# MarkJhonBao/InfantPoseEstimation_GaussianBias

Hardware: AMD Instinct MI355X
Metric: images/sec (train fwd+bwd) HRFormer-S 256x192 (higher is better)
Workload: dtype bf16; 1 GPU; HRFormer-small + fusion head, 256x192 -> 64x48, K=17, train step fwd+bwd+AdamW, DropPath 0.1, BN train; global_batch=64, per_gpu_batch=64, parallelism=dp1, launch=hipGraph replay, branches on concurrent HIP streams

## Files before the change

include/posekernels.h:

```cpp
#ifndef POSEKERNELS_H
#define POSEKERNELS_H

#include <stdint.h>

#ifdef __cplusplus
extern "C" {
#endif

#define PK_OK 0
#define PK_ERR_INVALID (-1)
#define PK_ERR_UNSUPPORTED (-2)

#define PK_DT_F32 0
#define PK_DT_BF16 1

int pk_version(void);
const char* pk_last_error_string(void);
int pk_marker(int id, void* stream);

int pk_gaussian_target(const float* keypoints, const float* visible, const float* lut, int lut_len,
                       float* target, float* weight, int B, int K, int Hh, int Wh,
                       double stride_x, double stride_y, double reach, int patch_n, int patch_c, void* stream);

int pk_dense_target(const float* keypoints, const float* visible, float* heatmaps, float* weights,
// ... 219 lines not shown
} PkConvDesc;
int pk_conv2d_group(const PkConvDesc* descs, int n, void* stream);
typedef struct PkBnFwdDesc {
    const void* raw; const float* stats_partial; const float* gamma; const float* beta;
    float* running_mean; float* running_var; int64_t* num_batches_tracked;
    const void* residual; void* y; float* save_mean; float* save_rstd; uint8_t* relu_mask ;
    int64_t rows; int tiles, C; float momentum, eps; int relu;
} PkBnFwdDesc;
int pk_bn_train_fwd_group(const PkBnFwdDesc* descs, int n, void* stream);
typedef struct PkBnBwdDesc {
    const void* dy; const void* y_act; const void* raw; const float* save_mean; const float* save_rstd; const float* gamma;
    float* partial; float* dgamma; float* dbeta; void* dx; void* dresidual; const uint8_t* relu_mask ;
    int64_t rows; int C; int relu;
} PkBnBwdDesc;
int pk_bn_bwd_group_blocks(int64_t rows);
int pk_bn_bwd_group(const PkBnBwdDesc* descs, int n, void* stream);
typedef struct PkFuseDesc {
    const void* inputs[4]; int in_h[4]; int in_w[4]; int n_inputs;
    void* out; const void* mask_y; int B, H, W, C, relu;
} PkFuseDesc;
int pk_fuse_sum_group(const PkFuseDesc* descs, int n, void* stream);
typedef struct PkUpBwdDesc {
    const void* dy; const void* mask_y; void* dsrc; int B, H, W, Hs, Ws, C;
} PkUpBwdDesc;
int pk_upsample_bwd_group(const PkUpBwdDesc* descs, int n, void* stream);
typedef struct PkWgradDesc {
    const void* x; const void* grad_out; float* workspace;
    int B, Hs, Ws, Ho, Wo, N, Cin, ksize, stride;
} PkWgradDesc;
int pk_wgrad_group_slices(int M, int N, int Cin, int ksize, int stride);
int pk_wgrad_group(const PkWgradDesc* descs, int n, void* stream);
int pk_sizeof_group_desc(int which);

int pk_conv_stats_rows(int B, int Hs, int Ws, int Cin, int Cout, int ksize, int stride, int Ho, int Wo);

int pk_linear_bf16(const void* x, const void* w, void* out, const float* bias, const void* residual, const float* res_scale,
                   const int32_t* a_rowmap, const int32_t* o_rowmap, void* preact_out, const void* gelu_grad_of,
                   int M, int N, int K, int rows_per_sample, int act, int out_fp32, void* stream);

int pk_rows_by_map(const void* src, void* dst, const int32_t* rowmap, int64_t n_rows, int row_bytes, int scatter, void* stream);
int pk_drop_path_f32(const float* x, const float* mask, float* out, int64_t batch, int64_t per_sample, float keep_prob, void* stream);

int pk_wgrad_slices(int M, int N, int Cin, int ksize, int stride, int Hs, int Ws, int flags);
int pk_wgrad_bf16(const void* x, const void* grad_out, float* workspace, float* dw, float* dbias, int n_bias,
                  const int32_t* a_rowmap, const int32_t* g_rowmap, const float* g_scale, int g_rows_per_sample, int M, int N,
                  int Cin, int ksize, int stride, int B, int Hs, int Ws, int Ho, int Wo, int out_layout, void* stream);

int pk_window_attn_fwd(const void* qkv, const float* rel_table, void* out, float* lse, int n_windows, int heads, int C,
                       float softmax_scale, void* stream);
int pk_window_attn_bwd_groups(int n_windows, int heads);
int pk_window_attn_bwd_ws_floats(int n_windows, int heads);
int pk_window_attn_bwd(const void* qkv, const float* rel_table, const void* fwd_out, const void* dout, const float* lse, void* dqkv,
                       float* dbias_partial, float* dtable, int n_windows, int heads, int C, float softmax_scale, void* stream);

int pk_sum_partials(const float* partial, int nb, int K, int stride, float* out, float scale, int accumulate, void* stream);
int pk_bn_finalize(const float* stats_partial, int tiles, int C, int count, const float* gamma, const float* beta,
                   float* running_mean, float* running_var, int64_t* num_batches_tracked, float momentum, float eps,
                   float* scale, float* shift, float* save_mean, float* save_rstd, void* stream);
int pk_bn_act(const void* x, const float* scale, const float* shift, const void* residual, void* y, int64_t rows, int C,
              int relu, uint8_t* relu_mask, void* stream);
int pk_bn_train_fwd(const void* raw, const float* stats_partial, int tiles, int C, int64_t rows, const float* gamma, const float* beta,
                    float* running_mean, float* running_var, int64_t* num_batches_tracked, float momentum, float eps, const void* residual,
                    void* y, float* save_mean, float* save_rstd, float* scale, float* shift, int relu, uint8_t* relu_mask, void* stream);
int pk_bn_bwd_blocks(int64_t rows);
int pk_bn_bwd(const void* dy, const void* y_act, const void* raw, const float* save_mean, const float* save_rstd,
              const float* gamma, float* partial, float* sums, float* dgamma, float* dbeta, void* dx, void* dresidual,
              int64_t rows, int C, int relu, const uint8_t* relu_mask, void* stream);
int pk_relu_bwd(const void* dy, const void* y, void* dx, int64_t numel, void* stream);

int pk_conv1x1_bn_supported(int64_t rows, int Cin, int Cout);
int pk_conv1x1_stats_rows(int64_t rows);
int pk_conv1x1_bn_bwd_rows(int64_t rows);
int pk_conv1x1_stats(const void* x, const void* w, float* stats_partial, int64_t rows, int Cin, int Cout, void* stream);
int pk_conv1x1_bn_act(const void* x, const void* w, const float* scale, const float* shift, const void* residual, void* y, int relu,
                      uint8_t* relu_mask, int64_t rows, int Cin, int Cout, void* stream);
int pk_conv1x1_bn_bwd_reduce(const void* dy, const void* x, const void* w, const float* save_mean, const float* save_rstd, float* partial,
                             int64_t rows, int Cin, int Cout, int relu, const uint8_t* relu_mask, void* stream);
int pk_conv1x1_bn_bwd_apply(const void* dy, const void* x, const void* w, const float* save_mean, const float* save_rstd, const float* gamma,
                            const float* sums, float inv_count, void* draw, void* dresidual, int64_t rows, int Cin, int Cout, int relu,
                            const uint8_t* relu_mask, void* stream);
int pk_conv1x1_bn_bwd(const void* dy, const void* x, const void* w, const float* save_mean, const float* save_rstd, const float* gamma,
                      float* partial, float* sums, float* dgamma, float* dbeta, void* draw, void* dresidual, int64_t rows, int Cin, int Cout,
                      int relu, const uint8_t* relu_mask, void* stream);
int pk_layernorm_fwd(const void* x, const float* gamma, const float* beta, void* y, float* save_mean, float* save_rstd,
                     int64_t rows, int C, int C_real, float eps, void* stream);
int pk_ln_bwd_blocks(int64_t rows);
int pk_layernorm_bwd(const void* dy, const void* x, const float* save_mean, const float* save_rstd, const float* gamma,
                     const void* dresidual, void* dx, float* partial, float* dgamma, float* dbeta, int64_t rows, int C, int C_real,
                     void* stream);
int pk_ln_mlp_supported(int C);
int pk_ln_mlp_hidden_slice(int C);
int pk_ln_mlp_slab_floats(int C);
int pk_ln_mlp_dx_blocks(int M, int C);
int pk_ln_mlp_dw_blocks(int M, int C);
int pk_ln_mlp_fwd(const void* x, const float* gamma, const float* beta, const void* w1, const float* b1, const void* w2,
                  const float* b2, const float* row_scale, void* y, int M, int C, int rows_per_sample, float eps, void* stream);
int pk_ln_mlp_wide_supported(int C, int hidden, int M);
int pk_ln_mlp_wide_fwd(const void* x, const float* gamma, const float* beta, const void* w1, const float* b1, const void* w2,
                       const float* b2, const float* row_scale, void* y, int M, int C, int c_real, int hidden, int rows_per_sample,
                       float eps, void* stream);
int pk_ln_mlp_bwd_dx(const void* dy, const void* x, const float* gamma, const float* beta, const void* w1, const float* b1,
                     const void* w1_t, const void* w2_t, const float* row_scale, void* dx, float* ln_partial, int M, int C,
                     int rows_per_sample, float eps, void* stream);
int pk_ln_mlp_bwd_dw(const void* dy, const void* x, const float* gamma, const float* beta, const void* w1, const float* b1,
                     const void* w2_t, const float* row_scale, float* slabs, int M, int C, int rows_per_sample, float eps,
                     void* stream);
int pk_attn_block_wide_supported(int C, int heads, int n_windows);
int pk_attn_block_wide_fwd(const void* x, const int32_t* rowmap, const float* gamma, const float* beta, const float* rel_table,
                           const void* wqkv, const float* bqkv, const void* wproj, const float* bproj, const float* row_scale,
                           void* y, int n_windows, int windows_per_sample, int heads, int C, int c_real, float softmax_scale,
                           float eps, void* stream);
int pk_attn_block_supported(int C, int heads);
int pk_attn_block_fwd(const void* x, const int32_t* rowmap, const float* gamma, const float* beta, const float* rel_table,
                      const void* wqkv, const float* bqkv, const void* wproj, const float* bproj, const float* row_scale,
                      void* y, void* o_save, float* lse, int n_windows, int windows_per_sample, int heads, int C, float eps,
                      void* stream);
int pk_attn_block_blocks(int n_windows);
int pk_attn_block_bwd(const void* dy, const void* x, const int32_t* rowmap, const float* gamma, const float* beta,
                      const float* rel_table, const void* wqkv, const float* bqkv, const void* wqkv_t, const void* wproj_t,
                      const float* row_scale, const void* o_saved, const float* lse, void* dx, void* dqkv, void* u_out,
                      float* ln_partial, float* rpb_partial, int n_windows, int windows_per_sample, int heads, int C, float eps,
                      void* stream);
int pk_colsum_bf16(const void* g, const int32_t* rowmap, const float* row_scale, int rows_per_sample, float* partial,
                   float* out, int64_t rows, int N, void* stream);
int pk_fuse_sum(const void* const* inputs, const int* in_h, const int* in_w, int n_inputs, void* out, int B, int H, int W,
                int C, int relu, void* stream);
int pk_upsample_bilinear_bwd(const void* dy, void* dsrc, int B, int H, int W, int Hs, int Ws, int C, void* stream);
int pk_nchw_f32_to_nhwc_bf16(const float* x, const float* softplus_out, void* y, int B, int Cin, int H, int W, int Cpad,
                             void* stream);
int pk_reduce_many_cols(void);
int pk_reduce_many(const void* desc_table, const int* block_desc, const int* block_first, int n_blocks, void* stream);
int pk_pack_weights(void* flat_dst_bf16, const void* desc_table, const int32_t* block_desc, const int32_t* block_first,
                    int n_blocks, void* stream);
int pk_embed_boxes(float* twin_base, const void* desc_table, const int* block_desc, const int* block_first, int n_blocks,
                   int direction, void* stream);

int pk_draw_shapes(void* images_u8, int N, int H, int W, const float* poses, const float* scores, const int32_t* image_index, int P,
                   int K, const int32_t* limbs, int L, const void* colors_u8, int C, const float* boxes,
                   const int32_t* box_image_index, int Q, int box_c0, int box_c1, int box_c2, int box_thickness,
                   float score_threshold, int point_radius, int line_thickness, void* stream);
int pk_heatmap_overlay_ws_floats(int N, int K, int h, int w, int H, int W);
int pk_heatmap_overlay(void* images_u8, const float* heatmaps, float alpha, const void* lut_u8, void* index_u8, float* ws, int N,
                       int K, int h, int w, int H, int W, void* stream);
int pk_heatmap_overlay_patches_ws_floats(int P, int K, int h, int w);
int pk_heatmap_overlay_patches(void* images_u8, const float* heatmaps, const int32_t* patch_image_index, const double* patch_matrix,
                               float alpha, const void* lut_u8, void* index_u8, void* cover_u8, float* ws, int N, int P, int K, int h,
                               int w, int H, int W, void* stream);

#ifdef __cplusplus
}
#endif
#endif
```

infantposeestimation_gaussianbias_amd/dispatch.py:

```python
import contextlib
import os

import torch

from . import nnops
from ._lib import PoseKernelError

_ACTIVE = []


def backend_for(model):
    ok = getattr(model, "_pk_supported", None)
    if ok is None:
        ok = nnops.supported(model)
        object.__setattr__(model, "_pk_supported", ok)
    if not ok:
        raise PoseKernelError(
            f"{type(model).__name__}: layer shapes outside the HIP kernels (channels must be multiples of 8, head_dim a multiple of 8 "
            "up to 64, window 7) and no 8-aligned padded twin could be built (models/padded.py); there is no fallback path")
    return nnops


def padded_twin(model):
    if getattr(model, "_pk_twin", None) is False:
        return None
    from .models import padded
    return padded.twin_for(model)


def backend_name(model) -> str:
    if torch.cuda.is_available() and padded_twin(model) is not None:
        return "hip (8-aligned padded twin)"
    backend_for(model)
    return "hip"


@contextlib.contextmanager
def scope(model):
    if _ACTIVE:
        yield _ACTIVE[-1]
        return
    ops = backend_for(model)
    _ACTIVE.append(ops)
    try:
        with nnops.use_weights(model):
            yield ops
            join_detached()
    finally:
        _ACTIVE.pop()


def ops():
    if not _ACTIVE:
        raise RuntimeError("network op called outside dispatch.scope(model)")
    return _ACTIVE[-1]


from .nnops import (backward_milestone, conv_bn_act, deconv_bn_relu, drop_scales, eval_drop_scales, exchange, exchange_output, head_out,
                    mlp_rows, residual_block, stochastic_depth, to_features, window_attention_tokens, window_block)


def to_public(x):
    ops()
    return x.permute(0, 3, 1, 2)


def from_public(x):
    ops()
    if x.dtype != nnops.ACT_DTYPE:
        B, C, H, W = x.shape
        if x.requires_grad and torch.is_grad_enabled() and C % 8 == 0:
            return x.permute(0, 2, 3, 1).to(nnops.ACT_DTYPE).contiguous()
        return nnops.to_features(x, cpad=-(-C // 8) * 8)
    return x.permute(0, 2, 3, 1).contiguous()


_SIDE = {}
_STREAMS_OFF = [False]
_REGION = [False]
_EVENTS = []


def set_streams(enabled: bool):
    _STREAMS_OFF[0] = not enabled


def set_region_mode(enabled: bool):
    _REGION[0] = bool(enabled)


def streams_enabled() -> bool:
    return (not _STREAMS_OFF[0]) and os.environ.get("POSE_STREAMS", "1") != "0" and torch.cuda.is_available()


def _side_stream(dev, i):
    key = (dev.index if dev.index is not None else torch.cuda.current_device(), i)
    if key not in _SIDE:
        _SIDE[key] = torch.cuda.Stream(device=dev)
    return _SIDE[key]


def join_side_streams(cur=None):
    cur = cur or torch.cuda.current_stream()
    for s in _SIDE.values():
        cur.wait_stream(s)


_DETACHED = []


def run_detached(fn, tensors):
    with torch.no_grad():
        if not streams_enabled() or _MARK:
            fn()
            return
        cur = torch.cuda.current_stream()
        s = _side_stream(cur.device, 7)
        _order(cur, s)
        with torch.cuda.stream(s):
            for t in tensors:
                t.record_stream(s)
            fn()
        _DETACHED.append(s)


def join_detached():
    if _DETACHED:
        cur = torch.cuda.current_stream()
        for s in _DETACHED:
            _order(s, cur)
        _DETACHED.clear()




def _tensors(obj):
    if torch.is_tensor(obj):
        yield obj
    elif isinstance(obj, (list, tuple)):
        for o in obj:
            yield from _tensors(o)
# ... 129 lines not shown
```

infantposeestimation_gaussianbias_amd/models/fusion_head.py:

```python
import math
from typing import Dict, Optional, Tuple

import torch
import torch.nn as nn

from .. import hipops
from .. import dispatch as nnops
from ._blocks import conv
from .losses import HardKeypointMining


class SoftArgmax2D(nn.Module):

    def __init__(self, beta: float = 1.0):
        super().__init__()
        self.beta = beta

    def forward(self, heatmaps: torch.Tensor) -> Tuple[torch.Tensor, torch.Tensor]:
        h = heatmaps.float()
        if torch.is_grad_enabled() and h.requires_grad:
            co, sc = hipops.softargmax(h)
            if self.beta != 1.0:
                co = hipops.softargmax(h * self.beta)[0]
            return co, sc
        one = torch.full((1,), 40.0, device=heatmaps.device)
        co, sc = hipops.softargmax_refine_decode(h, None, one, None, radius=0)
        if self.beta != 1.0:
            co, _ = hipops.softargmax_refine_decode((h * self.beta).contiguous(), None, one, None, radius=0)
        return co, sc


class LocalGaussianRefinement(nn.Module):

    def __init__(self, local_radius: int = 2):
        super().__init__()
        self.local_radius = local_radius

    @torch.no_grad()
    def forward(self, heatmaps: torch.Tensor, coarse_coords: torch.Tensor) -> torch.Tensor:
        return hipops.local_gaussian_refine(heatmaps.float(), coarse_coords.float(), self.local_radius)


class SubPixelRefinement(nn.Module):

    def __init__(self, beta: float = 1.0, local_radius: int = 2, fusion_alpha: float = 0.5):
        super().__init__()
        self.local_radius = local_radius
        self.soft_argmax = SoftArgmax2D(beta=beta)
        self.local_refine = LocalGaussianRefinement(local_radius=local_radius)
        self.alpha = nn.Parameter(torch.tensor(fusion_alpha))

    def forward(self, heatmaps):
        return hipops.softargmax_refine_decode(heatmaps.float(), None, self.alpha.detach(), None, self.local_radius)


def _branch(cin, hidden, cout):
    seq = nn.ModuleDict({"0": conv(cin, hidden, 3), "1": nn.BatchNorm2d(hidden), "3": nn.Conv2d(hidden, cout, 1)})
    return seq


class HeatmapRegressionHead(nn.Module):
    def __init__(self, in_channels: int, num_keypoints: int = 17, hidden_dim: int = 256, use_subpixel_refinement: bool = True):
        super().__init__()
        self.in_channels, self.num_keypoints, self.use_subpixel_refinement = in_channels, num_keypoints, use_subpixel_refinement
        self.shared_layers = nn.ModuleDict({"0": conv(in_channels, hidden_dim, 3), "1": nn.BatchNorm2d(hidden_dim),
                                            "3": conv(hidden_dim, hidden_dim, 3), "4": nn.BatchNorm2d(hidden_dim)})
        self.heatmap_branch = _branch(hidden_dim, hidden_dim, num_keypoints)
        self.offset_branch = _branch(hidden_dim, hidden_dim, num_keypoints * 2)
        self.variance_branch = _branch(hidden_dim, hidden_dim // 2, num_keypoints)
        if use_subpixel_refinement:
            self.subpixel_refine = SubPixelRefinement(1.0, 2, 0.5)
        self.fusion_weight = nn.Parameter(torch.tensor(0.5))
        for m in self.modules():
            if isinstance(m, nn.Conv2d):
                nn.init.kaiming_normal_(m.weight, mode="fan_out", nonlinearity="relu")
                if m.bias is not None:
                    nn.init.zeros_(m.bias)

    def forward(self, x: torch.Tensor) -> Dict[str, torch.Tensor]:
        with nnops.scope(self):
            return self._forward(x)

    def _forward(self, x: torch.Tensor) -> Dict[str, torch.Tensor]:
        tr = self.training
        x = nnops.from_public(x)
        s = self.shared_layers
        f = nnops.conv_bn_act(x, s["0"], s["1"], True, None, tr)
        f = nnops.conv_bn_act(f, s["3"], s["4"], True, None, tr)

        def make(br, softplus=False):
            def run(ins):
                t = nnops.conv_bn_act(ins[0], br["0"], br["1"], True, None, tr)
                return nnops.head_out(t, br["3"], softplus)
            return run

        heatmaps, offsets, variances = nnops.parallel([make(self.heatmap_branch), make(self.offset_branch), make(self.variance_branch, True)],
                                                      [[f], [f], [f]])
        B, _, H, W = offsets.shape
        return {"heatmaps": heatmaps, "offsets": offsets.view(B, self.num_keypoints, 2, H, W),
                "variances": variances, "fusion_weight": torch.sigmoid(self.fusion_weight)}

    @torch.no_grad()
    def decode(self, outputs: Dict[str, torch.Tensor], apply_offset: bool = True) -> Tuple[torch.Tensor, torch.Tensor]:
        hm = outputs["heatmaps"].float()
        if self.use_subpixel_refinement:
            alpha, radius = self.subpixel_refine.alpha.detach(), self.subpixel_refine.local_radius
        else:
            alpha, radius = torch.full((1,), 40.0, device=hm.device), 0
        if not apply_offset:
            return hipops.softargmax_refine_decode(hm, None, alpha, None, radius)
        fw = outputs["fusion_weight"].detach().float().reshape(1)
        raw = torch.log(fw / (1 - fw))
        return hipops.softargmax_refine_decode(hm, outputs["offsets"].float(), alpha, raw, radius)


_TERM = {"heatmap": 0, "offset": 1, "peak": 2, "variance": 3, "overlap": 4, "shape": 5}


def _lam(dev, thr=0.5, **terms):
    v = [0.0] * 6 + [float(thr)]
    for k, w in terms.items():
        v[_TERM[k]] = float(w)
    return torch.tensor(v, dtype=torch.float32, device=dev)


class GaussianDistributionConstraint(nn.Module):
    SKELETON = [(0, 1), (0, 2), (1, 3), (2, 4), (5, 6), (5, 7), (7, 9), (6, 8), (8, 10), (5, 11), (6, 12), (11, 12),
                (11, 13), (13, 15), (12, 14), (14, 16)]

    def __init__(self, target_sigma: float = 2.0, overlap_threshold: float = 0.5):
        super().__init__()
        self.target_sigma, self.overlap_threshold = target_sigma, overlap_threshold

    def _terms(self, heatmaps, coords, target_weight, pred_variances, **terms):
        return hipops.fusion_terms(_lam(heatmaps.device, self.overlap_threshold, **terms), hm=heatmaps, var=pred_variances, coords=coords,
                                   weight=target_weight, sigma_t=self.target_sigma)

    def compute_heatmap_variance(self, heatmaps: torch.Tensor, coords: torch.Tensor) -> torch.Tensor:
        return self._terms(heatmaps, coords, None, None)[1]

    def variance_alignment_loss(self, heatmaps, coords, target_weight, pred_variances: Optional[torch.Tensor] = None) -> torch.Tensor:
        return self._terms(heatmaps, coords, target_weight, pred_variances, variance=1.0)[0][3]

    def spatial_overlap_loss(self, heatmaps, target_weight) -> torch.Tensor:
        return self._terms(heatmaps, None, target_weight, None, overlap=1.0)[0][4]

    def distribution_shape_loss(self, heatmaps, target_weight) -> torch.Tensor:
        return self._terms(heatmaps, None, target_weight, None, shape=1.0)[0][5]

    def forward(self, heatmaps, coords, target_weight, pred_variances: Optional[torch.Tensor] = None) -> Dict[str, torch.Tensor]:
        v = self._terms(heatmaps, coords, target_weight, pred_variances, variance=1.0, overlap=1.0, shape=1.0)[0]
        return {"variance_loss": v[3], "overlap_loss": v[4], "shape_loss": v[5]}


class FusionPoseLoss(HardKeypointMining, nn.Module):
    NAMES = ("heatmap_loss", "offset_loss", "peak_loss", "variance_loss", "overlap_loss", "shape_loss", "total_loss")

    def __init__(self, heatmap_weight: float = 1.0, offset_weight: float = 1.0, peak_weight: float = 0.5,
                 variance_weight: float = 0.1, overlap_weight: float = 0.05, shape_weight: float = 0.05,
                 target_sigma: float = 2.0, use_target_weight: bool = True, ohkm_topk: int = 0, ohkm_weight: float = 1.0,
                 num_keypoints: Optional[int] = None):
        super().__init__()
        self._init_ohkm(ohkm_topk, num_keypoints, ohkm_weight)
        self.heatmap_weight, self.offset_weight, self.peak_weight = heatmap_weight, offset_weight, peak_weight
        self.variance_weight, self.overlap_weight, self.shape_weight = variance_weight, overlap_weight, shape_weight
        self.use_target_weight = use_target_weight
        self.gaussian_constraint = GaussianDistributionConstraint(target_sigma)
        self.soft_argmax = SoftArgmax2D()
        self.register_buffer("_lambdas", torch.tensor([heatmap_weight, offset_weight, peak_weight, variance_weight, overlap_weight, shape_weight,
                                                       self.gaussian_constraint.overlap_threshold], dtype=torch.float32), persistent=False)

    def heatmap_loss(self, pred, target, weight) -> torch.Tensor:
        return hipops.fusion_terms(_lam(pred.device, heatmap=1.0), hm=pred, target=target, weight=weight,
                                   use_target_weight=self.use_target_weight)[0][0]

    def offset_loss(self, pred_offsets, pred_coords, gt_coords, weight, input_size, heatmap_size) -> torch.Tensor:
# ... 34 lines not shown
```

infantposeestimation_gaussianbias_amd/nnops.py:

```python
import os

import numpy as np
import torch

from . import _lib
from ._lib import call, stream_ptr

BF16, F32, I32 = torch.bfloat16, torch.float32, torch.int32
ACT_DTYPE = BF16
WS = 7


def _e(shape, dtype, dev):
    return torch.empty(shape, dtype=dtype, device=dev)


_OBSERVER = [None]


class observe:

    def __init__(self, collector):
        self.collector = collector

# ... 598 lines not shown


class _BnActOnly(torch.autograd.Function):

    @staticmethod
    def forward(ctx, raw, part, gamma, beta, bn, relu, training):
        ctx.params = (gamma, beta)
        raw = raw.contiguous()
        y, mean, rstd = _bn_forward(raw, part, gamma, beta, bn, None, relu, training, None)
        ctx.save_for_backward(raw, y, mean, rstd, gamma)
        ctx.meta = (relu, training)
        return y

    @staticmethod
    def backward(ctx, dy):
        raw, y, mean, rstd, gamma = ctx.saved_tensors
        relu, training = ctx.meta
        draw, _, dgamma, dbeta = _bn_backward(dy.contiguous(), y, None, raw, mean, rstd, gamma, *ctx.params, relu, training, False)
        return draw, None, dgamma, dbeta, None, None, None


def deconv_bn_relu(x, deconv, bn, training):
    from . import hipops
    w = deconv.weight
    Cin, Cout, k, _ = w.shape
    if deconv.stride[0] != 2 or deconv.bias is not None or Cout % 8 or Cin % 8:
        raise _lib.PoseKernelError("deconv layer: stride-2 ConvTranspose2d without bias and channel counts that are multiples of 8")
    B, H, W, _ = x.shape
    raw_s, part = _ConvW.apply(x, _StackDeconv.apply(w))
    key = (B, H, W, str(x.device))
    if key not in _SHUFFLE_MAPS:
        b, oy, ox = torch.meshgrid(torch.arange(B), torch.arange(2 * H), torch.arange(2 * W), indexing="ij")
        m = (((b * H + oy // 2) * W + ox // 2) * 4 + (oy % 2) * 2 + (ox % 2)).reshape(-1)
        _SHUFFLE_MAPS[key] = m.to(torch.int32).to(x.device)
    raw = hipops.rows_by_map(raw_s.view(B * H * W * 4, Cout), _SHUFFLE_MAPS[key], B * 4 * H * W, False).view(B, 2 * H, 2 * W, Cout)
    t = part.shape[0]
    part4 = part.view(t, 2, 4, Cout).permute(0, 2, 1, 3).reshape(4 * t, 2, Cout).contiguous()
    return _BnActOnly.apply(raw, part4, bn.weight, bn.bias, bn, True, training)


class _HeadOut(torch.autograd.Function):
    @staticmethod
    def forward(ctx, x, weight, bias, softplus):
        ctx.params = (weight, bias)
        wc = _wc()
        wf, wd = wc.fwd[id(weight)], wc.dgrad[id(weight)]
        x = x.contiguous()
        B, H, W, Cin = x.shape
        N = weight.shape[0]
        out = _e((B, N, H, W), F32, x.device)
        call("pk_conv2d_nhwc", x, wf, out, None, bias, B, H, W, Cin, N, 1, 1, 0, H, W, 2 if softplus else 0, 2, None, stream_ptr())
        ctx.save_for_backward(x, out if softplus else x.new_empty(0), wd)
        ctx.meta = (softplus, N)
        return out

    @staticmethod
    def backward(ctx, dout):
        x, y, wd = ctx.saved_tensors
        softplus, N = ctx.meta
        B, H, W, Cin = x.shape
        Np = _up8(N)
        g = _e((B, H, W, Np), BF16, x.device)
        call("pk_nchw_f32_to_nhwc_bf16", dout.contiguous(), y if softplus else None, g, B, N, H, W, Np, stream_ptr())
        dx = _e((B, H, W, Cin), BF16, x.device)
        call("pk_conv2d_nhwc", g, wd, dx, None, None, B, H, W, Np, Cin, 1, 1, 0, H, W, 0, 0, None, stream_ptr())
        w, b = (_Dest(p) for p in ctx.params)
        geom = (B, H, W, H, W)
        if _deferrable(w, b):
            _wgrad(x, g, Np, Cin, 1, 1, geom, out=w.t, dbias=b.t, deferred=True, n_real=N)
            return dx, None, None, None
        db = _e((N,), F32, x.device)
        dw = _wgrad(x, g, Np, Cin, 1, 1, geom, dbias=db)[:N]
        if w.direct and b.direct:
            w.t.copy_(dw)
            b.t.copy_(db)
            return dx, None, None, None
        return dx, dw.contiguous(), db.contiguous(), None


def head_out(x, conv, softplus=False):
    return _HeadOut.apply(x, conv.weight, conv.bias, softplus)


_MAPS = {}


def window_rowmap(B, H, W, device):
    key = (B, H, W, str(device))
    if key not in _MAPS:
        nh, nw = -(-H // WS), -(-W // WS)
        ys = (torch.arange(nh)[:, None] * WS + torch.arange(WS)[None, :])
        xs = (torch.arange(nw)[:, None] * WS + torch.arange(WS)[None, :])
        yy = ys[:, None, :, None].expand(nh, nw, WS, WS)
        xx = xs[None, :, None, :].expand(nh, nw, WS, WS)
        pix = torch.where((yy < H) & (xx < W), yy * W + xx, torch.full_like(yy, -1)).reshape(-1)
        full = pix[None, :].repeat(B, 1)
        full = torch.where(full >= 0, full + torch.arange(B)[:, None] * (H * W), full)
        _MAPS[key] = (full.reshape(-1).to(torch.int32).to(device), nh * nw)
    return _MAPS[key]


def _layernorm(x2d, gamma, beta, c_real=0):
    M, C = x2d.shape
    y = _e((M, C), BF16, x2d.device)
    mean, rstd = _e((M,), F32, x2d.device), _e((M,), F32, x2d.device)
    call("pk_layernorm_fwd", x2d, gamma, beta, y, mean, rstd, M, C, c_real, 1e-5, stream_ptr())
    return y, mean, rstd


def _layernorm_bwd(dy, x2d, mean, rstd, gamma, dres, g_param=None, b_param=None, c_real=0):
    M, C = x2d.shape
    nb = _lib.lib.pk_ln_bwd_blocks(M)
    dx = _e((M, C), BF16, x2d.device)
    dg, db = _Dest(g_param, (C,), x2d.device), _Dest(b_param, (C,), x2d.device)
    deferred = _deferrable(dg, db)
    part = _workspace(dg.t, "ln", nb * 2 * C, deferred)
    call("pk_layernorm_bwd", dy, x2d, mean, rstd, gamma, dres, dx, part, None if deferred else dg.t, None if deferred else db.t, M, C, c_real,
         stream_ptr())
    if deferred:
        _reduce([_row((part, 0), (dg.t, 0), 2 * C, nb, C), _row((part, C), (db.t, 0), 2 * C, nb, C)], True)
    return dx, dg.grad(), db.grad()


def _linear(x, w, out_rows, N, K, bias=None, residual=None, res_scale=None, a_map=None, o_map=None, preact=None, gelu_of=None,
            M=None, rps=0, act=0):
    out = _e((out_rows, N), BF16, x.device)
    call("pk_linear_bf16", x, w, out, bias, residual, res_scale, a_map, o_map, preact, gelu_of, M if M is not None else out_rows, N, K,
         rps, act, 0, stream_ptr())
    return out


class _AttnHalf(torch.autograd.Function):

    @staticmethod
    def forward(ctx, x, g1, b1, table, wqkv, bqkv, wproj, bproj, scale1, heads, c_real=0, attn_scale=0.0):
        ctx.params = (g1, b1, table, wqkv, bqkv, wproj, bproj)
        ctx.pad = (c_real, attn_scale)
        wc = _wc()
        x = x.contiguous()
        B, H, W, C = x.shape
        M = B * H * W
        amap, nwin = window_rowmap(B, H, W, x.device)
        Mw = B * nwin * WS * WS
        x2 = x.view(M, C)
        u, mean, rstd = _layernorm(x2, g1, b1, c_real)
        qkv = _linear(u, wc.fwd[id(wqkv)], Mw, 3 * C, C, bias=bqkv, a_map=amap)
        o = _e((Mw, C), BF16, x.device)
        lse = _e((B * nwin * heads * WS * WS,), F32, x.device)
        call("pk_window_attn_fwd", qkv, table, o, lse, B * nwin, heads, C, attn_scale, stream_ptr())
        s1 = _scale(scale1)
        y = _linear(o, wc.fwd[id(wproj)], M, C, C, bias=bproj, residual=x2, res_scale=s1, o_map=amap, M=Mw, rps=H * W)
        ctx.save_for_backward(x2, u, mean, rstd, qkv, o, lse, g1, table, _stash(s1, x), wc.dgrad[id(wqkv)], wc.dgrad[id(wproj)], amap)
        ctx.meta = (B, H, W, C, heads, nwin)
        return y.view(B, H, W, C)

    @staticmethod
    def backward(ctx, dy):
        x2, u, mean, rstd, qkv, o, lse, g1, table, s1, wqkv_t, wproj_t, amap = ctx.saved_tensors
        B, H, W, C, heads, nwin = ctx.meta
        s1 = _unstash(s1)
        M, Mw = B * H * W, B * nwin * WS * WS
        dev = dy.device
        dy2 = dy.contiguous().view(M, C)
        pg1, pb1, ptab, pwqkv, pbqkv, pwproj, pbproj = ctx.params
        d_o = _linear(dy2, wproj_t, Mw, C, C, res_scale=s1, a_map=amap, rps=nwin * WS * WS)
        dwproj, dbproj = _linear_wgrad(pwproj, pbproj, o, dy2, C, C, g_map=amap, g_scale=s1, g_rps=H * W, M=Mw, win=(B, H, W))
# ... 478 lines not shown
```

Baseline: 4243 images/sec.

## Fuse head BN+ReLU with 1x1 output conv in forward and backward

Adds a HIP kernel that applies batch-norm scale/shift and ReLU to the raw conv output and immediately runs the small 1x1 output projection with MFMA. It writes the NCHW float heatmap plus the activation and ReLU mask in one pass. The backward kernel fuses the output-conv dgrad with the BN backward reduce and apply phases. This removes separate elementwise and GEMM launches and intermediate round trips for the three head branches. In exchange it adds a custom code path that is gated by row count and shape, and it is less tested than the generic ops.

```diff
diff --git a/include/posekernels.h b/include/posekernels.h
--- a/include/posekernels.h
+++ b/include/posekernels.h
@@ -325,6 +325,12 @@
 int pk_conv1x1_bn_bwd(const void* dy, const void* x, const void* w, const float* save_mean, const float* save_rstd, const float* gamma,
                       float* partial, float* sums, float* dgamma, float* dbeta, void* draw, void* dresidual, int64_t rows, int Cin, int Cout,
                       int relu, const uint8_t* relu_mask, void* stream);
+int pk_bn_out1x1_supported(int64_t rows, int C, int N);
+int pk_bn_out1x1_fwd(const void* raw, const float* scale, const float* shift, const void* w_fwd, const float* bias, void* t, float* out,
+                     uint8_t* relu_mask, int64_t rows, int C, int N, int hw, int softplus, void* stream);
+int pk_bn_out1x1_bwd(const void* g, const void* raw, const uint8_t* relu_mask, const void* w_dgrad, const float* save_mean,
+                     const float* save_rstd, const float* gamma, float* partial, float* sums, float* dgamma, float* dbeta, void* draw,
+                     int64_t rows, int C, int N, void* stream);
 int pk_layernorm_fwd(const void* x, const float* gamma, const float* beta, void* y, float* save_mean, float* save_rstd,
                      int64_t rows, int C, int C_real, float eps, void* stream);
 int pk_ln_bwd_blocks(int64_t rows);
diff --git a/infantposeestimation_gaussianbias_amd/csrc/pk_bn_out1x1.hip b/infantposeestimation_gaussianbias_amd/csrc/pk_bn_out1x1.hip
--- /dev/null
+++ b/infantposeestimation_gaussianbias_amd/csrc/pk_bn_out1x1.hip
@@ -0,0 +1,496 @@
+#include <stdlib.h>
+
+#include "pk_rowops.h"
+
+#define BO_ROWS 128
+#define BO_GRID 512
+#define BO_MIN_ROWS 32768
+#define BO_SMALL_ROWS 32768
+
+struct BnOutArgs {
+    const uint4* raw;
+    const uint16_t* w;
+    const uint16_t* g;
+    const uint8_t* mask_in;
+    uint8_t* mask_out;
+    const float* v0;
+    const float* v1;
+    const float* gamma;
+    const float* sums;
+    const float* bias;
+    float* out;
+    uint4* t_out;
+    uint4* draw;
+    float* part;
+    float inv_count;
+    int small;
+    int64_t rows;
+    int N, N8, hw, softplus;
+    int nb, rpb;
+};
+
+template <int C>
+struct BoGeom {
+    static constexpr int CPR = C / 8;
+    static constexpr int RPI = 64 / CPR;
+    static constexpr int NLD = 16 / RPI;
+    static constexpr int TP = C + 8;
+    static constexpr int RL = 256 / CPR;
+    static constexpr int TILE_BYTES = (16 * TP * 2 > RL * C * 4) ? 16 * TP * 2 : RL * C * 4;
+};
+
+__device__ __forceinline__ void bo_wave_sync() {
+    __builtin_amdgcn_fence(__ATOMIC_ACQ_REL, "wavefront");
+    __builtin_amdgcn_wave_barrier();
+}
+
+template <int C, int NB>
+__global__ void __launch_bounds__(256, 2) k_bn_out1x1_fwd(BnOutArgs p) {
+    using G = BoGeom<C>;
+    constexpr int CPR = G::CPR, RPI = G::RPI, NLD = G::NLD, TP = G::TP;
+    extern __shared__ __attribute__((aligned(16))) unsigned char bo_smem[];
+    uint16_t* sW = reinterpret_cast<uint16_t*>(bo_smem);
+    const int tid = threadIdx.x, lane = tid & 63, wave = tid >> 6;
+    uint16_t* tile = reinterpret_cast<uint16_t*>(bo_smem + NB * 16 * TP * 2) + wave * 16 * TP;
+    const int frow = lane & 15, fkc = lane >> 4;
+    const int lch = lane % CPR, lrw = lane / CPR;
+    const int64_t rows = p.rows;
+    const int ntiles = (int)((rows + BO_ROWS - 1) / BO_ROWS);
+    auto block_base = [&](int it) -> int64_t {
+        const int64_t t = (int64_t)blockIdx.x + (int64_t)(it >> 1) * gridDim.x;
+        return t < ntiles ? t * BO_ROWS + wave * 32 + (it & 1) * 16 : -1;
+    };
+    auto load_raw = [&](uint4 (&rv)[NLD], int64_t base) {
+#pragma unroll
+        for (int i = 0; i < NLD; ++i) {
+            const int64_t row = base + i * RPI + lrw;
+            rv[i] = make_uint4(0u, 0u, 0u, 0u);
+            if (base >= 0 && row < rows) rv[i] = p.raw[(size_t)row * CPR + lch];
+        }
+    };
+    uint4 rv[NLD], rn[NLD];
+    int64_t base = block_base(0);
+    load_raw(rv, base);
+    for (int i = tid; i < NB * 16 * CPR; i += 256) {
+        const int n = i / CPR, ch = i - n * CPR;
+        u32x4 v = {0u, 0u, 0u, 0u};
+        if (n < p.N) v = reinterpret_cast<const u32x4*>(p.w)[(size_t)n * CPR + ch];
+        *reinterpret_cast<u32x4*>(&sW[n * TP + ch * 8]) = v;
+    }
+    float sc[8], sh[8], bs[NB][4];
+#pragma unroll
+    for (int j = 0; j < 8; ++j) {
+        sc[j] = p.v0[lch * 8 + j];
+        sh[j] = p.v1[lch * 8 + j];
+    }
+#pragma unroll
+    for (int a = 0; a < NB; ++a)
+#pragma unroll
+        for (int r = 0; r < 4; ++r) {
+            const int n = a * 16 + fkc * 4 + r;
+            bs[a][r] = n < p.N ? p.bias[n] : 0.f;
+        }
+    __syncthreads();
+    for (int it = 0; base >= 0; ++it) {
+        const int64_t nbase = block_base(it + 1);
+        load_raw(rn, nbase);
+        bo_wave_sync();
+#pragma unroll
+        for (int i = 0; i < NLD; ++i) {
+            const int rl = i * RPI + lrw;
+            const int64_t row = base + rl;
+            uint4 o = make_uint4(0u, 0u, 0u, 0u);
+            if (row < rows) {
+                float v[8];
+                unpack8(rv[i], v);
+#pragma unroll
+                for (int j = 0; j < 8; ++j) v[j] = fmaxf(v[j] * sc[j] + sh[j], 0.f);
+                o = pack8(v);
+                p.t_out[(size_t)row * CPR + lch] = o;
+                p.mask_out[(size_t)row * CPR + lch] = (uint8_t)pos_mask8(o);
+            }
+            *reinterpret_cast<uint4*>(&tile[rl * TP + lch * 8]) = o;
+        }
+        bo_wave_sync();
+        f32x4 acc[NB];
+#pragma unroll
+        for (int a = 0; a < NB; ++a) acc[a] = (f32x4){0.f, 0.f, 0.f, 0.f};
+#pragma unroll
+        for (int ks = 0; ks < C / 32; ++ks) {
+            const bf16x8 tf = *reinterpret_cast<const bf16x8*>(&tile[frow * TP + (ks * 4 + fkc) * 8]);
+#pragma unroll
+            for (int a = 0; a < NB; ++a) {
+                const bf16x8 wf = *reinterpret_cast<const bf16x8*>(&sW[(a * 16 + frow) * TP + (ks * 4 + fkc) * 8]);
+                acc[a] = __builtin_amdgcn_mfma_f32_16x16x32_bf16(wf, tf, acc[a], 0, 0, 0);
+            }
+        }
+        const int64_t row = base + frow;
+        if (row < rows) {
+            const int bb = (int)(row / p.hw), pix = (int)(row - (int64_t)bb * p.hw);
+            float* o = p.out + (size_t)bb * p.N * p.hw + pix;
+#pragma unroll
+            for (int a = 0; a < NB; ++a)
+#pragma unroll
+                for (int r = 0; r < 4; ++r) {
+                    const int n = a * 16 + fkc * 4 + r;
+                    if (n < p.N) {
+                        float v = acc[a][r] + bs[a][r];
+                        if (p.softplus) v = softplus_(v);
+                        o[(size_t)n * p.hw] = v;
+                    }
+                }
+        }
+#pragma unroll
+        for (int i = 0; i < NLD; ++i) rv[i] = rn[i];
+        base = nbase;
+    }
+}
+
+template <int MODE, int C, int KP>
+__global__ void __launch_bounds__(256, MODE == 1 ? 1 : 2) k_bn_out1x1_bwd(BnOutArgs p) {
+    using G = BoGeom<C>;
+    constexpr int CPR = G::CPR, RPI = G::RPI, NLD = G::NLD, TP = G::TP, RL = G::RL;
+    constexpr int WP = KP + 8, KS = KP / 32;
+    extern __shared__ __attribute__((aligned(16))) unsigned char bo_smem[];
+    uint16_t* sWd = reinterpret_cast<uint16_t*>(bo_smem);
+    float* sVec = reinterpret_cast<float*>(bo_smem + C * WP * 2);
+    unsigned char* tiles = bo_smem + C * WP * 2 + 5 * C * 4;
+    const int tid = threadIdx.x, lane = tid & 63, wave = tid >> 6;
+    uint16_t* tile = reinterpret_cast<uint16_t*>(tiles + wave * G::TILE_BYTES);
+    const int frow = lane & 15, fkc = lane >> 4;
+    const int lch = lane % CPR, lrw = lane / CPR;
+    const int64_t rows = p.rows;
+    const int ntiles = (int)((rows + BO_ROWS - 1) / BO_ROWS);
+    const int bpu = (p.rpb + 15) / 16;
+    const int total_it = MODE == 1 ? ((p.nb + 4 * (int)gridDim.x - 1) / (4 * (int)gridDim.x)) * bpu : 0;
+    auto position = [&](int it, int& unit, int64_t& base, int64_t& end) {
+        base = end = 0;
+        unit = -1;
+        if (MODE == 1) {
+            const int q = it / bpu, k = it - q * bpu;
+            const int u = ((int)blockIdx.x + q * (int)gridDim.x) * 4 + wave;
+            if (it < total_it && u < p.nb) {
+                unit = u;
+                base = (int64_t)u * p.rpb + 16 * k;
+                end = min(rows, (int64_t)(u + 1) * p.rpb);
+            }
+        } else {
+            const int64_t t = (int64_t)blockIdx.x + (int64_t)(it >> 1) * gridDim.x;
+            if (t < ntiles) {
+                unit = 0;
+                base = t * BO_ROWS + wave * 32 + (it & 1) * 16;
+                end = rows;
+            }
+        }
+    };
+    struct Block {
+        uint4 rv[NLD];
+        uint32_t mv[NLD];
+        bf16x8 gf[KS];
+    };
+    auto load_block = [&](Block& b, int64_t base, int64_t end) {
+#pragma unroll
+        for (int i = 0; i < NLD; ++i) {
+            const int64_t row = base + i * RPI + lrw;
+            b.rv[i] = make_uint4(0u, 0u, 0u, 0u);
+            b.mv[i] = 0u;
+            if (row < end) {
+                b.rv[i] = p.raw[(size_t)row * CPR + lch];
+                b.mv[i] = p.mask_in[(size_t)row * CPR + lch];
+            }
+        }
+#pragma unroll
+        for (int ks = 0; ks < KS; ++ks) {
+            const int64_t row = base + frow;
+            b.gf[ks] = (bf16x8){0, 0, 0, 0, 0, 0, 0, 0};
+            if (row < end && (ks * 4 + fkc) * 8 < p.N8) b.gf[ks] = *reinterpret_cast<const bf16x8*>(p.g + (size_t)row * p.N8 + (ks * 4 + fkc) * 8);
+        }
+    };
+    Block cur, nxt, nx2;
+    int unit, nunit;
+    int64_t base, end, nbase, nend;
+    position(0, unit, base, end);
+    load_block(cur, base, end);
+    position(1, nunit, nbase, nend);
+    if (MODE == 1) load_block(nxt, nbase, nend);
+    {
+        const int wch = p.N8 / 8;
+        for (int i = tid; i < C * (KP / 8); i += 256) {
+            const int c = i / (KP / 8), ch = i - c * (KP / 8);
+            u32x4 v = {0u, 0u, 0u, 0u};
+            if (ch < wch) v = reinterpret_cast<const u32x4*>(p.w)[(size_t)c * wch + ch];
+            *reinterpret_cast<u32x4*>(&sWd[c * WP + ch * 8]) = v;
+        }
+        for (int c = tid; c < C; c += 256) {
+            sVec[c] = p.v0[c];
+            sVec[C + c] = p.v1[c];
+            if (MODE == 2) {
+                sVec[2 * C + c] = p.gamma[c];
+                sVec[3 * C + c] = p.sums[c];
+                sVec[4 * C + c] = p.sums[C + c];
+            }
+        }
+    }
+    float s1[4][8], s2[4][8];
+    if (MODE == 1) {
+#pragma unroll
+        for (int s = 0; s < 4; ++s)
+#pragma unroll
+            for (int j = 0; j < 8; ++j) s1[s][j] = s2[s][j] = 0.f;
+    }
+    __syncthreads();
+    for (int it = 0; MODE == 1 ? it < total_it : unit >= 0; ++it) {
+        int n2unit = -1;
+        int64_t n2base = 0, n2end = 0;
+        if (MODE == 1) {
+            position(it + 2, n2unit, n2base, n2end);
+            load_block(nx2, n2base, n2end);
+        } else {
+            load_block(nxt, nbase, nend);
+        }
+        bo_wave_sync();
+#pragma unroll
+        for (int cg = 0; cg < C / 64; ++cg) {
+            f32x4 acc[4];
+#pragma unroll
+            for (int a = 0; a < 4; ++a) acc[a] = (f32x4){0.f, 0.f, 0.f, 0.f};
+#pragma unroll
+            for (int ks = 0; ks < KS; ++ks)
+#pragma unroll
+                for (int a = 0; a < 4; ++a) {
+                    const bf16x8 wf = *reinterpret_cast<const bf16x8*>(&sWd[(cg * 64 + a * 16 + frow) * WP + (ks * 4 + fkc) * 8]);
+                    acc[a] = __builtin_amdgcn_mfma_f32_16x16x32_bf16(wf, cur.gf[ks], acc[a], 0, 0, 0);
+                }
+#pragma unroll
+            for (int a = 0; a < 4; ++a) {
+                const u32x2 d = {pack_bf16x2(acc[a][0] + 0.f, acc[a][1] + 0.f), pack_bf16x2(acc[a][2] + 0.f, acc[a][3] + 0.f)};
+                *reinterpret_cast<u32x2*>(&tile[frow * TP + cg * 64 + a * 16 + fkc * 4]) = d;
+            }
+        }
+        bo_wave_sync();
+        {
+            float mu[8], rs[8], va[8], vb[8], vc[8];
+            {
+                const int c0 = lch * 8;
+#pragma unroll
+                for (int j = 0; j < 8; ++j) {
+                    mu[j] = sVec[c0 + j];
+                    rs[j] = sVec[C + c0 + j];
+                    va[j] = MODE == 2 ? sVec[2 * C + c0 + j] : 0.f;
+                    vb[j] = MODE == 2 ? sVec[3 * C + c0 + j] : 0.f;
+                    vc[j] = MODE == 2 ? sVec[4 * C + c0 + j] : 0.f;
+                }
+            }
+#pragma unroll
+            for (int i = 0; i < NLD; ++i) {
+                const int rl = i * RPI + lrw;
+                const int64_t row = base + rl;
+                const uint16_t* cell = &tile[rl * TP + lch * 8];
+                if (row >= end) continue;
+                float g[8], xr[8];
+                unpack8(*reinterpret_cast<const uint4*>(cell), g);
+                unpack8(cur.rv[i], xr);
+                const uint32_t mb = cur.mv[i];
+                if (MODE == 1) {
+#pragma unroll
+                    for (int j = 0; j < 8; ++j) {
+                        const float gg = ((mb >> j) & 1u) ? g[j] : 0.f;
+                        s1[i & 3][j] += gg;
+                        s2[i & 3][j] += gg * (xr[j] - mu[j]) * rs[j];
+                    }
+                } else {
+                    float o[8];
+                    if (p.small) {
+#pragma unroll
+                        for (int j = 0; j < 8; ++j) {
+                            const float gg = ((mb >> j) & 1u) ? g[j] : 0.f;
+                            const float gm = va[j] * rs[j], t1 = vb[j] * p.inv_count, t2 = vc[j] * p.inv_count;
+                            const float xh = (xr[j] - mu[j]) * rs[j];
+                            o[j] = gm * (gg - t1 - xh * t2);
+                        }
+                    } else {
+#pragma unroll
+                        for (int j = 0; j < 8; ++j) {
+                            const float gg = ((mb >> j) & 1u) ? g[j] : 0.f;
+                            const float xh = (xr[j] - mu[j]) * rs[j];
+                            o[j] = va[j] * rs[j] * (gg - vb[j] * p.inv_count - xh * vc[j] * p.inv_count);
+                        }
+                    }
+                    p.draw[(size_t)row * CPR + lch] = pack8(o);
+                }
+            }
+        }
+        if (MODE == 1) {
+            if (unit >= 0 && it - (it / bpu) * bpu == bpu - 1) {
+                float* stage = reinterpret_cast<float*>(tile);
+                float* dst = p.part + (size_t)unit * 2 * C;
+#pragma unroll
+                for (int h = 0; h < 2; ++h) {
+                    bo_wave_sync();
+#pragma unroll
+                    for (int s = 0; s < 4; ++s)
+#pragma unroll
+                        for (int j = 0; j < 8; ++j) {
+                            stage[(s * RPI + lrw) * C + lch * 8 + j] = h ? s2[s][j] : s1[s][j];
+                            if (h) s1[s][j] = s2[s][j] = 0.f;
+                        }
+                    bo_wave_sync();
+#pragma unroll
+                    for (int q = 0; q < C / 64; ++q) {
+                        float a = 0.f;
+#pragma unroll
+                        for (int k = 0; k < RL; ++k) a += stage[k * C + q * 64 + lane];
+                        dst[h * C + q * 64 + lane] = a;
+                    }
+                }
+                bo_wave_sync();
+            }
+        }
+        cur = nxt;
+        unit = nunit;
+        base = nbase;
+        end = nend;
+        if (MODE == 1) {
+            nxt = nx2;
+            nunit = n2unit;
+            nbase = n2base;
+            nend = n2end;
+        } else {
+            position(it + 2, nunit, nbase, nend);
+        }
+    }
+}
+
+__global__ void __launch_bounds__(256) k_bn_out1x1_sum_small(const float* __restrict__ part, int nb, int C, float* __restrict__ sums,
+                                                             float* __restrict__ dbeta, float* __restrict__ dgamma) {
+    __shared__ double sh1[8][32], sh2[8][32];
+    const int c0 = (int)blockIdx.x * 32;
+    const int cl = threadIdx.x & 31, pl = threadIdx.x >> 5, c = c0 + cl;
+    double a = 0.0, b = 0.0;
+    if (c < C)
+        for (int t = pl; t < nb; t += 8) {
+            a += (double)part[(size_t)t * 2 * C + c];
+            b += (double)part[(size_t)t * 2 * C + C + c];
+        }
+    sh1[pl][cl] = a;
+    sh2[pl][cl] = b;
+    __syncthreads();
+    if (threadIdx.x < 32 && c < C) {
+        a = b = 0.0;
+#pragma unroll
+        for (int k = 0; k < 8; ++k) {
+            a += sh1[k][cl];
+            b += sh2[k][cl];
+        }
+        sums[c] = (float)a;
+        sums[C + c] = (float)b;
+        dbeta[c] = (float)a;
+        dgamma[c] = (float)b;
+    }
+}
+
+static inline int bo_grid(int64_t want) {
+    const char* cap = getenv("PK_BN_OUT1X1_MAX_GRID");
+    int64_t lim = BO_GRID;
+    if (cap && atoi(cap) >= 1 && atoi(cap) < BO_GRID) lim = atoi(cap);
+    if (want > lim) want = lim;
+    return (int)(want < 1 ? 1 : want);
+}
+static inline bool bo_shape_ok(int64_t rows, int C, int N) { return rows > 0 && rows < (1 << 30) && (C == 256 || C == 128) && N >= 1 && N <= 48; }
+extern "C" int pk_bn_out1x1_supported(int64_t rows, int C, int N) {
+    const char *on = getenv("PK_BN_OUT1X1"), *mr = getenv("PK_BN_OUT1X1_MIN_ROWS");
+    if (on && on[0] == '0') return 0;
+    int64_t min_rows = BO_MIN_ROWS;
+    if (mr && atoll(mr) >= 1) min_rows = atoll(mr);
+    return (bo_shape_ok(rows, C, N) && rows >= min_rows) ? 1 : 0;
+}
+static inline bool bo_aligned(const void* a, const void* b = nullptr, const void* c = nullptr, const void* d = nullptr) {
+    return (((uintptr_t)a | (uintptr_t)b | (uintptr_t)c | (uintptr_t)d) & 15) == 0;
+}
+#define BO_CHECK_SHAPE(who)                                                     \
+    PK_REQUIRE(rows > 0 && rows < (1 << 30) && N > 0, who ": bad sizes");       \
+    PK_SUPPORTED(bo_shape_ok(rows, C, N), who ": built for C = 128 / 256 channels and N <= 48 outputs (got %d -> %d)", C, N)
+
+static int bo_launch(void (*kernel)(BnOutArgs), bool& attr_set, int grid, int lds, const BnOutArgs& a, hipStream_t st, const char* who) {
+    const hipError_t e = attr_set ? hipSuccess : hipFuncSetAttribute((const void*)kernel, hipFuncAttributeMaxDynamicSharedMemorySize, lds);
+    if (e != hipSuccess) return pk_set_error("%s: cannot reserve %d bytes of LDS: %s", who, lds, hipGetErrorString(e)), (int)e;
+    attr_set = true;
+    hipLaunchKernelGGL(kernel, dim3((unsigned)grid), dim3(256), lds, st, a);
+    return pk_launch_status(who);
+}
+template <int C, int NB>
+static int bo_fwd(const BnOutArgs& a, hipStream_t st, const char* who) {
+    static bool attr_set = false;
+    const int lds = NB * 16 * BoGeom<C>::TP * 2 + 4 * 16 * BoGeom<C>::TP * 2;
+    return bo_launch(k_bn_out1x1_fwd<C, NB>, attr_set, bo_grid((a.rows + BO_ROWS - 1) / BO_ROWS), lds, a, st, who);
+}
+template <int MODE, int C, int KP>
+static int bo_bwd(const BnOutArgs& a, hipStream_t st, const char* who) {
+    const int lds = C * (KP + 8) * 2 + 5 * C * 4 + 4 * BoGeom<C>::TILE_BYTES;
+    const int grid = MODE == 1 ? bo_grid((a.nb + 3) / 4) : bo_grid((a.rows + BO_ROWS - 1) / BO_ROWS);
+    static bool attr_set = false;
+    return bo_launch(k_bn_out1x1_bwd<MODE, C, KP>, attr_set, grid, lds, a, st, who);
+}
+template <int MODE>
+static int bo_bwd_any(const BnOutArgs& a, int C, hipStream_t st, const char* who) {
+    if (C == 256) return a.N <= 32 ? bo_bwd<MODE, 256, 32>(a, st, who) : bo_bwd<MODE, 256, 64>(a, st, who);
+    return a.N <= 32 ? bo_bwd<MODE, 128, 32>(a, st, who) : bo_bwd<MODE, 128, 64>(a, st, who);
+}
+
+extern "C" int pk_bn_out1x1_fwd(const void* raw, const float* scale, const float* shift, const void* w_fwd, const float* bias, void* t, float* out,
+                                uint8_t* relu_mask, int64_t rows, int C, int N, int hw, int softplus, void* stream) {
+    PK_REQUIRE(raw && scale && shift && w_fwd && bias && t && out && relu_mask, "pk_bn_out1x1_fwd: null pointer");
+    BO_CHECK_SHAPE("pk_bn_out1x1_fwd");
+    PK_REQUIRE(hw > 0 && rows % hw == 0, "pk_bn_out1x1_fwd: rows = %lld is no multiple of the plane size %d", (long long)rows, hw);
+    PK_REQUIRE(bo_aligned(raw, w_fwd, t), "pk_bn_out1x1_fwd: raw, t and the weight must be 16-byte aligned");
+    BnOutArgs a{};
+    a.raw = (const uint4*)raw;
+    a.w = (const uint16_t*)w_fwd;
+    a.v0 = scale;
+    a.v1 = shift;
+    a.bias = bias;
+    a.out = out;
+    a.t_out = (uint4*)t;
+    a.mask_out = relu_mask;
+    a.rows = rows;
+    a.N = N;
+    a.hw = hw;
+    a.softplus = softplus ? 1 : 0;
+    hipStream_t st = (hipStream_t)stream;
+    const char* who = "pk_bn_out1x1_fwd";
+    if (C == 256) return N <= 32 ? bo_fwd<256, 2>(a, st, who) : bo_fwd<256, 3>(a, st, who);
+    return N <= 32 ? bo_fwd<128, 2>(a, st, who) : bo_fwd<128, 3>(a, st, who);
+}
+
+extern "C" int pk_bn_out1x1_bwd(const void* g, const void* raw, const uint8_t* relu_mask, const void* w_dgrad, const float* save_mean,
+                                const float* save_rstd, const float* gamma, float* partial, float* sums, float* dgamma, float* dbeta, void* draw,
+                                int64_t rows, int C, int N, void* stream) {
+    PK_REQUIRE(g && raw && relu_mask && w_dgrad && save_mean && save_rstd && gamma && partial && sums && dgamma && dbeta && draw,
+               "pk_bn_out1x1_bwd: null pointer");
+    BO_CHECK_SHAPE("pk_bn_out1x1_bwd");
+    PK_REQUIRE(bo_aligned(g, raw, w_dgrad, draw), "pk_bn_out1x1_bwd: tensors must be 16-byte aligned");
+    hipStream_t st = (hipStream_t)stream;
+    BnOutArgs a{};
+    a.raw = (const uint4*)raw;
+    a.w = (const uint16_t*)w_dgrad;
+    a.g = (const uint16_t*)g;
+    a.mask_in = relu_mask;
+    a.v0 = save_mean;
+    a.v1 = save_rstd;
+    a.part = partial;
+    a.rows = rows;
+    a.N = N;
+    a.N8 = (N + 7) / 8 * 8;
+    a.nb = pk_bn_bwd_blocks(rows);
+    a.rpb = (int)((rows + a.nb - 1) / a.nb);
+    if (int rc = bo_bwd_any<1>(a, C, st, "pk_bn_out1x1_bwd (reduce)")) return rc;
+    const int small = rows <= BO_SMALL_ROWS;
+    if (small) hipLaunchKernelGGL(k_bn_out1x1_sum_small, dim3((unsigned)((C + 31) / 32)), dim3(256), 0, st, partial, a.nb, C, sums, dbeta, dgamma);
+    else sum_partials_launch(partial, a.nb, 2 * C, 2 * C, sums, 1.f, 0, dbeta, dgamma, C, st);
+    a.gamma = gamma;
+    a.sums = sums;
+    a.inv_count = 1.f / (float)rows;
+    a.small = small;
+    a.draw = (uint4*)draw;
+    return bo_bwd_any<2>(a, C, st, "pk_bn_out1x1_bwd (apply)");
+}
diff --git a/infantposeestimation_gaussianbias_amd/dispatch.py b/infantposeestimation_gaussianbias_amd/dispatch.py
--- a/infantposeestimation_gaussianbias_amd/dispatch.py
+++ b/infantposeestimation_gaussianbias_amd/dispatch.py
@@ -56,7 +56,7 @@
     return _ACTIVE[-1]
 
 
-from .nnops import (backward_milestone, conv_bn_act, deconv_bn_relu, drop_scales, eval_drop_scales, exchange, exchange_output, head_out,
+from .nnops import (backward_milestone, conv_bn_act, conv_bn_act_out, deconv_bn_relu, drop_scales, eval_drop_scales, exchange, exchange_output, head_out,
                     mlp_rows, residual_block, stochastic_depth, to_features, window_attention_tokens, window_block)
 
 
diff --git a/infantposeestimation_gaussianbias_amd/models/fusion_head.py b/infantposeestimation_gaussianbias_amd/models/fusion_head.py
--- a/infantposeestimation_gaussianbias_amd/models/fusion_head.py
+++ b/infantposeestimation_gaussianbias_amd/models/fusion_head.py
@@ -90,8 +90,7 @@
 
         def make(br, softplus=False):
             def run(ins):
-                t = nnops.conv_bn_act(ins[0], br["0"], br["1"], True, None, tr)
-                return nnops.head_out(t, br["3"], softplus)
+                return nnops.conv_bn_act_out(ins[0], br["0"], br["1"], br["3"], softplus, tr)
             return run
 
         heatmaps, offsets, variances = nnops.parallel([make(self.heatmap_branch), make(self.offset_branch), make(self.variance_branch, True)],
diff --git a/infantposeestimation_gaussianbias_amd/nnops.py b/infantposeestimation_gaussianbias_amd/nnops.py
--- a/infantposeestimation_gaussianbias_amd/nnops.py
+++ b/infantposeestimation_gaussianbias_amd/nnops.py
@@ -704,6 +704,72 @@
     return _HeadOut.apply(x, conv.weight, conv.bias, softplus)
 
 
+class _ConvBnActOut(torch.autograd.Function):
+
+    @staticmethod
+    def forward(ctx, x, weight, gamma, beta, out_weight, out_bias, bn, softplus):
+        ctx.params = (weight, gamma, beta, out_weight, out_bias)
+        wc = _wc()
+        wf, wd = wc.fwd[id(weight)], wc.dgrad[id(weight)]
+        owf, owd = wc.fwd[id(out_weight)], wc.dgrad[id(out_weight)]
+        Cout, ksize, N = weight.shape[0], weight.shape[2], out_weight.shape[0]
+        x = x.contiguous()
+        B, Hs, Ws, Cin, Ho, Wo = _conv_geometry(x, ksize, 1)
+        M, dev = B * Ho * Wo, x.device
+        wc.bn_eval.pop(id(bn), None)
+        raw, part = _conv_raw(x, wf, Cout, ksize, 1, True)
+        scale, shift, mean, rstd = (_e((Cout,), F32, dev) for _ in range(4))
+        call("pk_bn_finalize", part, part.shape[0], Cout, M, gamma, beta, bn.running_mean, bn.running_var, bn.num_batches_tracked, 0.1, 1e-5,
+             scale, shift, mean, rstd, stream_ptr())
+        mask = _e((M * Cout // 8,), torch.uint8, dev)
+        t = _e((B, Ho, Wo, Cout), BF16, dev)
+        out = _e((B, N, Ho, Wo), F32, dev)
+        call("pk_bn_out1x1_fwd", raw, scale, shift, owf, out_bias, t, out, mask, M, Cout, N, Ho * Wo, 1 if softplus else 0, stream_ptr())
+        ctx.save_for_backward(x, raw, t, mask, mean, rstd, gamma, wd, owd, out if softplus else x.new_empty(0))
+        ctx.meta = (softplus, N, ksize, (B, Hs, Ws, Ho, Wo), Cout)
+        return out
+
+    @staticmethod
+    def backward(ctx, dout):
+        x, raw, t, mask, mean, rstd, gamma, wd, owd, y = ctx.saved_tensors
+        softplus, N, ksize, (B, Hs, Ws, Ho, Wo), Cout = ctx.meta
+        w_p, g_p, b_p, ow_p, ob_p = ctx.params
+        Cin, M, dev = x.shape[-1], B * Ho * Wo, x.device
+        Np = _up8(N)
+        g = _e((B, Ho, Wo, Np), BF16, dev)
+        call("pk_nchw_f32_to_nhwc_bf16", dout.contiguous(), y if softplus else None, g, B, N, Ho, Wo, Np, stream_ptr())
+        ow, ob = _Dest(ow_p), _Dest(ob_p)
+        geom = (B, Ho, Wo, Ho, Wo)
+        if _deferrable(ow, ob):
+            _wgrad(t, g, Np, Cout, 1, 1, geom, out=ow.t, dbias=ob.t, deferred=True, n_real=N)
+            dow = dob = None
+        else:
+            dob = _e((N,), F32, dev)
+            dow = _wgrad(t, g, Np, Cout, 1, 1, geom, dbias=dob)[:N]
+            if ow.direct and ob.direct:
+                ow.t.copy_(dow)
+                ob.t.copy_(dob)
+                dow = dob = None
+            else:
+                dow, dob = dow.contiguous(), dob.contiguous()
+        part, sums = _e((_lib.lib.pk_bn_bwd_blocks(M), 2, Cout), F32, dev), _e((2 * Cout,), F32, dev)
+        dgamma, dbeta = _Dest(g_p), _Dest(b_p)
+        draw = _e((B, Ho, Wo, Cout), BF16, dev)
+        call("pk_bn_out1x1_bwd", g, raw, mask, owd, mean, rstd, gamma, part, sums, dgamma.t, dbeta.t, draw, M, Cout, N, stream_ptr())
+        dx = _conv_dgrad(draw, wd, Cin, ksize, 1, (Hs, Ws)) if ctx.needs_input_grad[0] else None
+        w = _Dest(w_p)
+        _wgrad(x, draw, Cout, Cin, ksize, 1, (B, Hs, Ws, Ho, Wo), out=w.t, deferred=_deferrable(w))
+        return dx, w.grad(), dgamma.grad(), dbeta.grad(), dow, dob, None, None
+
+
+def conv_bn_act_out(x, conv, bn, out_conv, softplus=False, training=False):
+    Cin = conv.weight.shape[1]
+    if (training and torch.is_grad_enabled() and _OBSERVER[0] is None and conv.stride[0] == 1 and out_conv.bias is not None and
+            x.shape[-1] == Cin and _lib.lib.pk_bn_out1x1_supported(x.shape[0] * x.shape[1] * x.shape[2], conv.weight.shape[0], out_conv.weight.shape[0])):
+        return _ConvBnActOut.apply(x, conv.weight, bn.weight, bn.bias, out_conv.weight, out_conv.bias, bn, softplus)
+    return head_out(conv_bn_act(x, conv, bn, True, None, training), out_conv, softplus)
+
+
 _MAPS = {}
 
 
```

New measurement: 4300 images/sec (median of 6 runs). +1.3%, better.
